# iwbn/flow-supervisor

Hardware: AMD Instinct MI355X
Metric: image-pairs/s fwd+bwd, 12 GRU iters, 436x1024 (higher is better)
Workload: dtype f32 (bf16x3 products); 1 GPU; RAFT full, 440x1024 (Sintel 436x1024 padded), 12 GRU iters, 4 pairs/GPU, train step = fwd + sequence loss + bwd + RCCL all-reduce + clip + AdamW; global_batch=4, parallelism=dp1, launch=hipGraph replay of the whole step

## Files before the change

### flow_supervisor_amd/csrc/conv_small.hip

```cpp
#include "common.hpp"
#include <cstddef>

namespace {


constexpr int SMALL_RUN = 16;
constexpr int SMALL_RUN_FWD = 8;
constexpr int SMALL_CHUNK = 8;

constexpr unsigned SM_OOB = 0x80000000u;
__device__ __forceinline__ __amdgpu_buffer_rsrc_t sm_rsrc(const void* p) {
  const uint64_t u = reinterpret_cast<uint64_t>(p);
  const unsigned lo = __builtin_amdgcn_readfirstlane((unsigned)u), hi = __builtin_amdgcn_readfirstlane((unsigned)(u >> 32));
  return __builtin_amdgcn_make_buffer_rsrc(reinterpret_cast<void*>((uint64_t)hi << 32 | lo), 0, 0x7fffffff, 0x00020000);
}

template <int KC, int NOUT, int KH, int KW>
__global__ __launch_bounds__(256) void conv_small_fwd_kernel(const float* __restrict__ x, int ld, int C,
                                                             const float* __restrict__ w, const float* __restrict__ bias,
                                                             float* __restrict__ out, int64_t obs, int64_t ocs, int64_t ops,
                                                             int B, int H, int W) {
  static_assert(KH == 3 && KW == 3, "sliding window written for 3 x 3");
  const int lane = threadIdx.x & 63;
  constexpr int taps = 9;
  const int HW = H * W;
  f32x4 wr[NOUT][taps][KC];
#pragma unroll
  for (int o = 0; o < NOUT; ++o)
#pragma unroll
    for (int kc = 0; kc < KC; ++kc) {
      const int c = kc * 256 + lane * 4;
      float buf[36];
#pragma unroll
      for (int q = 0; q < 9; ++q) {
        const f32x4 v = c < C ? *reinterpret_cast<const f32x4*>(w + ((int64_t)o * C + c) * taps + 4 * q) : f32x4{0.f, 0.f, 0.f, 0.f};
        buf[4 * q] = v[0]; buf[4 * q + 1] = v[1]; buf[4 * q + 2] = v[2]; buf[4 * q + 3] = v[3];
      }
#pragma unroll
      for (int t = 0; t < taps; ++t) wr[o][t][kc] = f32x4{buf[t], buf[9 + t], buf[18 + t], buf[27 + t]};
    }
  const int rpr = (W + SMALL_RUN_FWD - 1) / SMALL_RUN_FWD;
  const int64_t nrun = (int64_t)B * H * rpr;
  const int64_t wave = (int64_t)blockIdx.x * 4 + (threadIdx.x >> 6), nwaves = (int64_t)gridDim.x * 4;
  const f32x4 zero = {0.f, 0.f, 0.f, 0.f};
  for (int64_t run = wave; run < nrun; run += nwaves) {
    const int x0 = (int)(run % rpr) * SMALL_RUN_FWD;
    const int64_t by = run / rpr;
    const int y = (int)(by % H), b = (int)(by / H);
    const int n = W - x0 < SMALL_RUN_FWD ? W - x0 : SMALL_RUN_FWD;
    const float* img = x + (int64_t)b * HW * ld;
    const __amdgpu_buffer_rsrc_t rs = sm_rsrc(img);
    auto load_col = [&](int xs, f32x4 (&col)[3][KC]) {
#pragma unroll
      for (int r = 0; r < 3; ++r) {
        const int yy = y + r - 1;
        const bool in = (unsigned)yy < (unsigned)H && (unsigned)xs < (unsigned)W;
#pragma unroll
        for (int kc = 0; kc < KC; ++kc) {
          const int c = kc * 256 + lane * 4;
          col[r][kc] = __builtin_bit_cast(f32x4, __builtin_amdgcn_raw_buffer_load_b128(rs, (in && c < C) ? (unsigned)((yy * W + xs) * ld + c) * 4u : SM_OOB, 0, 0));
        }
      }
    };
    f32x4 c0[3][KC], c1[3][KC], cn[SMALL_RUN_FWD][3][KC];
    load_col(x0 - 1, c0);
    load_col(x0, c1);
#pragma unroll
    for (int i = 0; i < SMALL_RUN_FWD; ++i) load_col(x0 + i + 1, cn[i]);
#pragma unroll
    for (int i = 0; i < SMALL_RUN_FWD; ++i) {
      if (i < n) {
        float acc[NOUT];
#pragma unroll
        for (int o = 0; o < NOUT; ++o) {
          f32x4 a4 = zero;
#pragma unroll
          for (int r = 0; r < 3; ++r)
#pragma unroll
            for (int kc = 0; kc < KC; ++kc) {
              a4 += c0[r][kc] * wr[o][3 * r + 0][kc];
              a4 += c1[r][kc] * wr[o][3 * r + 1][kc];
              a4 += cn[i][r][kc] * wr[o][3 * r + 2][kc];
            }
          acc[o] = (a4[0] + a4[1]) + (a4[2] + a4[3]);
        }
#pragma unroll
        for (int o = 0; o < NOUT; ++o) {
#pragma unroll
          for (int sft = 32; sft > 0; sft >>= 1) acc[o] += __shfl_xor(acc[o], sft, 64);
        }
        if (lane == 0) {
          const int pix = y * W + x0 + i;
#pragma unroll
          for (int o = 0; o < NOUT; ++o) out[b * obs + o * ocs + pix * ops] = acc[o] + (bias ? bias[o] : 0.f);
        }
      }
#pragma unroll
      for (int r = 0; r < 3; ++r)
#pragma unroll
        for (int kc = 0; kc < KC; ++kc) { c0[r][kc] = c1[r][kc]; c1[r][kc] = cn[i][r][kc]; }
    }
  }
}

constexpr int SMALL_MAX_SEG = 16;
struct SmallWgradArgs {
  const float* dy[SMALL_MAX_SEG]; const float* x[SMALL_MAX_SEG]; int nseg;
  int ldy, ldx, C, B, H, W, KH, KW, Ktot;
  float* dwpk; float* dbias;
};

template <int KC, int NOUT, int KH, int KW>
__global__ __launch_bounds__(256) void conv_small_wgrad_kernel(SmallWgradArgs a) {
  __shared__ float red[4][64 * 4];
  const int lane = threadIdx.x & 63, wv = threadIdx.x >> 6;
  constexpr int taps = KH * KW;
  const int HW = a.H * a.W;
  f32x4 acc[NOUT][taps][KC];
#pragma unroll
  for (int o = 0; o < NOUT; ++o)
#pragma unroll
    for (int t = 0; t < taps; ++t)
#pragma unroll
      for (int kc = 0; kc < KC; ++kc) acc[o][t][kc] = f32x4{0.f, 0.f, 0.f, 0.f};
  float bsum[NOUT];
#pragma unroll
  for (int o = 0; o < NOUT; ++o) bsum[o] = 0.f;
  static_assert(KH == 3 && KW == 3, "sliding window written for 3 x 3");
  const int64_t wave = (int64_t)blockIdx.x * 4 + wv, nwaves = (int64_t)gridDim.x * 4;
  const auto* karg = (const char __attribute__((address_space(4)))*)__builtin_amdgcn_kernarg_segment_ptr();
  typedef const float* fptr;
  const int rpr = (a.W + SMALL_RUN - 1) / SMALL_RUN;
  const int64_t nrun = (int64_t)a.B * a.H * rpr;
  for (int seg = 0; seg < a.nseg; ++seg) {
    const float* dy = ((const fptr __attribute__((address_space(4)))*)(karg + offsetof(SmallWgradArgs, dy)))[seg];
    const float* x = ((const fptr __attribute__((address_space(4)))*)(karg + offsetof(SmallWgradArgs, x)))[seg];
    for (int64_t run = wave; run < nrun; run += nwaves) {
      const int x0 = (int)(run % rpr) * SMALL_RUN;
      const int64_t by = run / rpr;
      const int y = (int)(by % a.H), b = (int)(by / a.H);
      const int n = a.W - x0 < SMALL_RUN ? a.W - x0 : SMALL_RUN;
      const float* img = x + (int64_t)b * HW * a.ldx;
      const __amdgpu_buffer_rsrc_t rs = sm_rsrc(img);
      auto load_col = [&](int xs, f32x4 (&col)[3][KC]) {
#pragma unroll
        for (int r = 0; r < 3; ++r) {
          const int yy = y + r - 1;
          const bool in = (unsigned)yy < (unsigned)a.H && (unsigned)xs < (unsigned)a.W;
#pragma unroll
          for (int kc = 0; kc < KC; ++kc) {
            const int c = kc * 256 + lane * 4;
            col[r][kc] = __builtin_bit_cast(f32x4, __builtin_amdgcn_raw_buffer_load_b128(rs, (in && c < a.C) ? (unsigned)((yy * a.W + xs) * a.ldx + c) * 4u : SM_OOB, 0, 0));
          }
        }
      };
      f32x4 c0[3][KC], c1[3][KC];
      load_col(x0 - 1, c0);
      load_col(x0, c1);
      for (int i0 = 0; i0 < n; i0 += SMALL_CHUNK) {
        f32x4 cn[SMALL_CHUNK][3][KC];
        float g[SMALL_CHUNK][NOUT];
#pragma unroll
        for (int i = 0; i < SMALL_CHUNK; ++i) {
          load_col(x0 + i0 + i + 1, cn[i]);
          const int64_t m = (int64_t)b * HW + (int64_t)y * a.W + x0 + i0 + (i0 + i < n ? i : 0);
#pragma unroll
          for (int o = 0; o < NOUT; ++o) g[i][o] = i0 + i < n ? dy[m * a.ldy + o] : 0.f;
        }
#pragma unroll
        for (int i = 0; i < SMALL_CHUNK; ++i) {
#pragma unroll
          for (int o = 0; o < NOUT; ++o) bsum[o] += g[i][o];
#pragma unroll
          for (int r = 0; r < 3; ++r)
#pragma unroll
            for (int kc = 0; kc < KC; ++kc)
#pragma unroll
              for (int o = 0; o < NOUT; ++o) {
                acc[o][3 * r + 0][kc] += g[i][o] * c0[r][kc];
                acc[o][3 * r + 1][kc] += g[i][o] * c1[r][kc];
                acc[o][3 * r + 2][kc] += g[i][o] * cn[i][r][kc];
              }
#pragma unroll
          for (int r = 0; r < 3; ++r)
#pragma unroll
            for (int kc = 0; kc < KC; ++kc) { c0[r][kc] = c1[r][kc]; c1[r][kc] = cn[i][r][kc]; }
        }
      }
    }
  }
  const int cpad = ((a.C + 31) / 32) * 32;
#pragma unroll
  for (int o = 0; o < NOUT; ++o)
#pragma unroll
    for (int t = 0; t < taps; ++t) {
#pragma unroll
      for (int kc = 0; kc < KC; ++kc) {
        __syncthreads();
#pragma unroll
        for (int i = 0; i < 4; ++i) red[wv][lane * 4 + i] = acc[o][t][kc][i];
        __syncthreads();
        const int c = kc * 256 + threadIdx.x;
        if (c < a.C && threadIdx.x < 256) {
          const float s = (red[0][threadIdx.x] + red[1][threadIdx.x]) + (red[2][threadIdx.x] + red[3][threadIdx.x]);
          atomicAdd(a.dwpk + (int64_t)o * a.Ktot + t * cpad + c, s);
        }
      }
    }
  if (a.dbias && lane == 0) {
#pragma unroll
    for (int o = 0; o < NOUT; ++o) atomicAdd(a.dbias + o, bsum[o]);
  }
}

constexpr int SMALL_RUN_DG = 16;
template <int N>
__global__ __launch_bounds__(256) void conv_small_dgrad_kernel(const float* __restrict__ dy, int ldy, const float* __restrict__ w_oihw,
                                                               float* __restrict__ dx, int lddx, const float* __restrict__ relu_src,
                                                               int ldm, int C, int B, int H, int W) {
  static_assert(N == 2, "two output channels");
  const int lane = threadIdx.x & 63;
  const int c0 = lane * 4;
  const bool on = c0 < C;
  float wr[N][4][9];
#pragma unroll
  for (int o = 0; o < N; ++o)
#pragma unroll
    for (int k = 0; k < 4; ++k)
#pragma unroll
      for (int t = 0; t < 9; ++t) wr[o][k][t] = (on && c0 + k < C) ? w_oihw[((int64_t)o * C + c0 + k) * 9 + t] : 0.f;
  const int runs_per_row = (W + SMALL_RUN_DG - 1) / SMALL_RUN_DG;
  const int64_t nrun = (int64_t)B * H * runs_per_row;
  const int nwave = gridDim.x * 4;
  for (int64_t run = blockIdx.x * 4 + (threadIdx.x >> 6); run < nrun; run += nwave) {
    const int64_t ru = __builtin_amdgcn_readfirstlane((int)run);
    const int xr = (int)(ru % runs_per_row), row = (int)(ru / runs_per_row), y = row % H, b = row / H;
    const int x0 = xr * SMALL_RUN_DG, x1 = min(W, x0 + SMALL_RUN_DG);
    const float* dyb = dy + (int64_t)b * H * W * ldy;
    float g[3][3][N];
    auto col = [&](int x, float (&gc)[3][N]) {
#pragma unroll
      for (int j = 0; j < 3; ++j) {
        const int yy = y + j - 1;
        const bool ok = (unsigned)yy < (unsigned)H && (unsigned)x < (unsigned)W;
        const float* p = dyb + (int64_t)((ok ? yy : y) * W + (ok ? x : x0)) * ldy;
#pragma unroll
        for (int o = 0; o < N; ++o) gc[j][o] = ok ? p[o] : 0.f;
      }
    };
    col(x0 - 1, g[0]);
    col(x0, g[1]);
    for (int x = x0; x < x1; ++x) {
      col(x + 1, g[2]);
      if (on) {
        const int64_t pix = ((int64_t)b * H + y) * W + x;
        f32x4 acc = {0.f, 0.f, 0.f, 0.f};
#pragma unroll
        for (int ky = 0; ky < 3; ++ky)
#pragma unroll
          for (int kx = 0; kx < 3; ++kx)
#pragma unroll
            for (int o = 0; o < N; ++o) {
              const float gv = g[2 - kx][2 - ky][o];
#pragma unroll
              for (int k = 0; k < 4; ++k) acc[k] += wr[o][k][ky * 3 + kx] * gv;
            }
        if (relu_src) {
          const f32x4 m = gload4(relu_src + pix * ldm + c0);
#pragma unroll
          for (int k = 0; k < 4; ++k) acc[k] = m[k] > 0.f ? acc[k] : 0.f;
        }
        gstore4(dx + pix * lddx + c0, acc);
      }
#pragma unroll
      for (int j = 0; j < 3; ++j)
#pragma unroll
        for (int o = 0; o < N; ++o) { g[0][j][o] = g[1][j][o]; g[1][j][o] = g[2][j][o]; }
    }
  }
}

}

extern "C" int fsraft_conv_small_fwd(const float* x, int ld, int C, const float* w_oihw, const float* bias, float* out,
                                     int64_t obs, int64_t ocs, int64_t ops, int N, int B, int H, int W, int KH, int KW,
                                     hipStream_t s) {
  if (!x || !w_oihw || !out || N != 2 || C < 4 || C > 512 || C % 4 || ld % 4 || KH != 3 || KW != 3 || B < 1 || ((uintptr_t)w_oihw % 16)) return FS_ERR_ARG;
  const int64_t M = (int64_t)B * H * W;
  const int64_t nrun = (int64_t)B * H * ((W + SMALL_RUN_FWD - 1) / SMALL_RUN_FWD);
  int blocks = (int)((nrun + 3) / 4);
  if (blocks > 2048) blocks = 2048;
  (void)M;
  if (C <= 256) hipLaunchKernelGGL((conv_small_fwd_kernel<1, 2, 3, 3>), dim3(blocks), dim3(256), 0, s, x, ld, C, w_oihw, bias, out, obs, ocs, ops, B, H, W);
  else hipLaunchKernelGGL((conv_small_fwd_kernel<2, 2, 3, 3>), dim3(blocks), dim3(256), 0, s, x, ld, C, w_oihw, bias, out, obs, ocs, ops, B, H, W);
  return fs_launch_status();
}

extern "C" int fsraft_conv_small_wgrad(const float* const* dy, const float* const* x, int nseg, int ldy, int ldx, int C,
                                       float* dwpk, float* dbias, int N, int B, int H, int W, int KH, int KW, hipStream_t s) {
  if (!dy || !x || !dwpk || nseg < 1 || N != 2 || C < 4 || C > 512 || C % 4 || ldx % 4 || KH != 3 || KW != 3) return FS_ERR_ARG;
  for (int base = 0; base < nseg; base += SMALL_MAX_SEG) {
    SmallWgradArgs a{};
    a.nseg = nseg - base < SMALL_MAX_SEG ? nseg - base : SMALL_MAX_SEG;
    for (int i = 0; i < a.nseg; ++i) { a.dy[i] = dy[base + i]; a.x[i] = x[base + i]; if (!a.dy[i] || !a.x[i]) return FS_ERR_ARG; }
    a.ldy = ldy; a.ldx = ldx; a.C = C; a.B = B; a.H = H; a.W = W; a.KH = KH; a.KW = KW;
    a.Ktot = KH * KW * (((C + 31) / 32) * 32); a.dwpk = dwpk; a.dbias = dbias;
    if (C <= 256) hipLaunchKernelGGL((conv_small_wgrad_kernel<1, 2, 3, 3>), dim3(512), dim3(256), 0, s, a);
    else hipLaunchKernelGGL((conv_small_wgrad_kernel<2, 2, 3, 3>), dim3(512), dim3(256), 0, s, a);
    const int rc = fs_launch_status();
    if (rc) return rc;
  }
  return FS_OK;
}

extern "C" int fsraft_conv_small_dgrad(const float* dy, int ldy, const float* w_oihw, float* dx, int lddx, const float* relu_src, int ldm,
                                       int C, int N, int B, int H, int W, int KH, int KW, hipStream_t s) {
  if (!dy || !w_oihw || !dx || N != 2 || C < 4 || C > 256 || C % 4 || lddx % 4 || ldy < 2 || KH != 3 || KW != 3 || B < 1 ||
      ((uintptr_t)dx % 16) || (relu_src && (ldm % 4 || ((uintptr_t)relu_src % 16))))
    return FS_ERR_ARG;
  const int64_t nrun = (int64_t)B * H * ((W + SMALL_RUN_DG - 1) / SMALL_RUN_DG);
  if (nrun >= ((int64_t)1 << 31)) return FS_ERR_ARG;
  int blocks = (int)((nrun + 3) / 4);
  if (blocks > 4096) blocks = 4096;
  hipLaunchKernelGGL((conv_small_dgrad_kernel<2>), dim3(blocks), dim3(256), 0, s, dy, ldy, w_oihw, dx, lddx, relu_src, ldm, C, B, H, W);
  return fs_launch_status();
}
```

### flow_supervisor_amd/csrc/stem.hip

```cpp
#include "common.hpp"
#include "gemm_core_split.hpp"

namespace {

typedef unsigned u32x4 __attribute__((ext_vector_type(4)));

constexpr unsigned ST_OOB = 0x80000000u;
__device__ __forceinline__ __amdgpu_buffer_rsrc_t st_rsrc(const void* p) {
  const uint64_t u = reinterpret_cast<uint64_t>(p);
  const unsigned lo = __builtin_amdgcn_readfirstlane((unsigned)u), hi = __builtin_amdgcn_readfirstlane((unsigned)(u >> 32));
  return __builtin_amdgcn_make_buffer_rsrc(reinterpret_cast<void*>((uint64_t)hi << 32 | lo), 0, 0x7fffffff, 0x00020000);
}

constexpr int ST_TW = 32;
constexpr int ST_K = 192;
constexpr int ST_PC = 72;

struct StemArgs {
  const float* x;
  const float* w;
  const float* bias;
  float* out;
  const float* dy;
  float* scratch;
  int B, H, W, Ho, Wo, N, tx, ty, ntiles;
};

__device__ __forceinline__ void split1(float v, unsigned short& hi, unsigned short& lo) {
  const __bf16 h = (__bf16)v;
  hi = __builtin_bit_cast(unsigned short, h);
  lo = __builtin_bit_cast(unsigned short, (__bf16)(v - (float)h));
}

constexpr int SF_TH = 8, SF_PR = 2 * SF_TH + 6, SF_WPITCH = 400;
constexpr int SF_WBYTES = 64 * SF_WPITCH, SF_PBYTES = 3 * SF_PR * ST_PC * 2, SF_NCH = (3 * SF_PR * ST_PC + 511) / 512;

__global__ __launch_bounds__(512) void stem_fwd_kernel(const StemArgs a) {
  __shared__ __attribute__((aligned(16))) char lds[2 * SF_WBYTES + 4 * SF_PBYTES];
  char* wh = lds;
  char* wl = lds + SF_WBYTES;
  char* pbuf = lds + 2 * SF_WBYTES;
  const int lane = threadIdx.x & 63, wave = threadIdx.x >> 6, l31 = lane & 31, lh = lane >> 5;
  for (int e = threadIdx.x; e < 64 * ST_K; e += 512) {
    const int n = e / ST_K, k = e - n * ST_K, c = k >> 6, ky = (k >> 3) & 7, kx = k & 7;
    const float v = (n < a.N && ky < 7 && kx < 7) ? a.w[((n * 3 + c) * 7 + ky) * 7 + kx] : 0.f;
    unsigned short h, l;
    split1(v, h, l);
    *reinterpret_cast<unsigned short*>(wh + n * SF_WPITCH + k * 2) = h;
    *reinterpret_cast<unsigned short*>(wl + n * SF_WPITCH + k * 2) = l;
  }
  const int nb = (a.N + 31) >> 5;
  const int tpi = a.tx * a.ty;
  float rp[SF_NCH];
  int pos[SF_NCH];
#pragma unroll
  for (int j = 0; j < SF_NCH; ++j) {
    const int e = threadIdx.x + 512 * j;
    const int c = e / (SF_PR * ST_PC), r = e - c * (SF_PR * ST_PC), py = r / ST_PC, px = r - py * ST_PC;
    pos[j] = e < 3 * SF_PR * ST_PC ? c << 16 | py << 8 | px : -1;
  }
  auto fetch = [&](int tile) {
    const int b = tile / tpi, tr = tile - b * tpi, oy0 = (tr / a.tx) * SF_TH, ox0 = (tr % a.tx) * ST_TW;
    const int iy0 = 2 * oy0 - 3, ix0 = 2 * ox0 - 3;
    const __amdgpu_buffer_rsrc_t rs = st_rsrc(a.x + (int64_t)b * 3 * a.H * a.W);
#pragma unroll
    for (int j = 0; j < SF_NCH; ++j) {
      const int c = pos[j] >> 16, iy = iy0 + ((pos[j] >> 8) & 255), ix = ix0 + (pos[j] & 255);
      const bool ok = pos[j] >= 0 && (unsigned)iy < (unsigned)a.H && (unsigned)ix < (unsigned)a.W;
      rp[j] = __builtin_bit_cast(float, __builtin_amdgcn_raw_buffer_load_b32(rs, ok ? (unsigned)((c * a.H + iy) * a.W + ix) * 4u : ST_OOB, 0, 0));
    }
  };
  auto stage = [&](char* ph) {
#pragma unroll
    for (int j = 0; j < SF_NCH; ++j) {
      const int e = threadIdx.x + 512 * j;
      if (e < 3 * SF_PR * ST_PC) {
        unsigned short h, l;
        split1(rp[j], h, l);
        *reinterpret_cast<unsigned short*>(ph + e * 2) = h;
        *reinterpret_cast<unsigned short*>(ph + SF_PBYTES + e * 2) = l;
      }
    }
  };
  const float bv0 = (a.bias && l31 < a.N) ? a.bias[l31] : 0.f, bv1 = (a.bias && 32 + l31 < a.N) ? a.bias[32 + l31] : 0.f;
  if ((int)blockIdx.x < a.ntiles) {
    fetch(blockIdx.x);
    stage(pbuf);
  }
  __syncthreads();
  int it = 0;
  for (int tile = blockIdx.x; tile < a.ntiles; tile += gridDim.x, ++it) {
    const int b = tile / tpi, tr = tile - b * tpi, oy0 = (tr / a.tx) * SF_TH, ox0 = (tr % a.tx) * ST_TW;
    const char* ph = pbuf + (it & 1) * 2 * SF_PBYTES;
    const char* pl = ph + SF_PBYTES;
    const bool more = tile + (int)gridDim.x < a.ntiles;
    if (more) fetch(tile + gridDim.x);
    f32x16 acc[2];
#pragma unroll
    for (int j = 0; j < 2; ++j)
#pragma unroll
      for (int r = 0; r < 16; ++r) acc[j][r] = 0.f;
#pragma unroll
    for (int s = 0; s < ST_K / 16; ++s) {
      const int g = 2 * s + lh, c = g >> 3, ky = g & 7;
      const int ao = ((c * SF_PR + 2 * wave + ky) * ST_PC + 2 * l31) * 2;
      u32x4 ahv, alv;
#pragma unroll
      for (int i = 0; i < 4; ++i) {
        ahv[i] = *reinterpret_cast<const unsigned*>(ph + ao + 4 * i);
        alv[i] = *reinterpret_cast<const unsigned*>(pl + ao + 4 * i);
      }
      const bf16x8 ah = __builtin_bit_cast(bf16x8, ahv), al = __builtin_bit_cast(bf16x8, alv);
#pragma unroll
      for (int j = 0; j < 2; ++j) {
        if (j < nb) {
          const int bo = (j * 32 + l31) * SF_WPITCH + (s * 16 + lh * 8) * 2;
          const bf16x8 bh = *reinterpret_cast<const bf16x8*>(wh + bo), bl = *reinterpret_cast<const bf16x8*>(wl + bo);
          acc[j] = __builtin_amdgcn_mfma_f32_32x32x16_bf16(al, bh, acc[j], 0, 0, 0);
          acc[j] = __builtin_amdgcn_mfma_f32_32x32x16_bf16(ah, bl, acc[j], 0, 0, 0);
          acc[j] = __builtin_amdgcn_mfma_f32_32x32x16_bf16(ah, bh, acc[j], 0, 0, 0);
        }
      }
      if (s & 1) __builtin_amdgcn_sched_barrier(0);
    }
    if (more) stage(pbuf + ((it + 1) & 1) * 2 * SF_PBYTES);
    const int oy = oy0 + wave;
    if (oy < a.Ho) {
      const __amdgpu_buffer_rsrc_t ro = st_rsrc(a.out + (int64_t)b * a.Ho * a.Wo * a.N);
      const int oxl = ox0 + 4 * lh;
#pragma unroll
      for (int j = 0; j < 2; ++j) {
        const int n = j * 32 + l31;
        if (j < nb) {
          const float bv = j ? bv1 : bv0;
          const unsigned vo = n < a.N ? (unsigned)((oy * a.Wo + oxl) * a.N + n) * 4u : ST_OOB;
#pragma unroll
          for (int r = 0; r < 16; ++r) {
            const int dx = (r & 3) + 8 * (r >> 2);
            __builtin_amdgcn_raw_buffer_store_b32(__builtin_bit_cast(unsigned, acc[j][r] + bv), ro, oxl + dx < a.Wo ? vo : ST_OOB,
                                                  (unsigned)(dx * a.N) * 4u, 0);
          }
        }
      }
    }
    __syncthreads();
  }
}

constexpr int SW_TH = 1, SW_PX = SW_TH * ST_TW, SW_PR = 2 * SW_TH + 6, SW_NDY = SW_PX * 16 / 512;
constexpr int SW_DYPITCH = 64 * 2 + 64, SW_IMPITCH = ST_K * 2 + 64;
constexpr int SW_DYPLANE = SW_PX * SW_DYPITCH, SW_IMPLANE = SW_PX * SW_IMPITCH, SW_PATCH = 3 * SW_PR * ST_PC * 4;
constexpr int SW_NCHP = (3 * SW_PR * ST_PC + 511) / 512;

__global__ __launch_bounds__(512, 2) void stem_wgrad_kernel(const StemArgs a) {
  constexpr int SW_LDS = 2 * SW_DYPLANE + 2 * SW_IMPLANE + SW_PATCH > 64 * ST_K * 4 ? 2 * SW_DYPLANE + 2 * SW_IMPLANE + SW_PATCH : 64 * ST_K * 4;
  __shared__ __attribute__((aligned(16))) char lds[SW_LDS];
  char* dyh = lds;
  char* imh = lds + 2 * SW_DYPLANE;
  float* patch = reinterpret_cast<float*>(lds + 2 * SW_DYPLANE + 2 * SW_IMPLANE);
  const int lane = threadIdx.x & 63, wave = threadIdx.x >> 6;
  const int kg = wave >> 2, mi = wave & 1, ns = (wave >> 1) & 1;
  const int lh = lane >> 5, gb = (lane >> 4) & 1, q = (lane & 15) >> 2, p4 = lane & 3, l31 = lane & 31;
  const int tpi = a.tx * a.ty;
  f32x16 acc[3];
#pragma unroll
  for (int j = 0; j < 3; ++j)
#pragma unroll
    for (int r = 0; r < 16; ++r) acc[j][r] = 0.f;

  float rdy[4 * SW_NDY], rp[SW_NCHP];
  int pos[SW_NCHP];
#pragma unroll
  for (int j = 0; j < SW_NCHP; ++j) {
    const int e = threadIdx.x + 512 * j;
    const int c = e / (SW_PR * ST_PC), r = e - c * (SW_PR * ST_PC), py = r / ST_PC, pxx = r - py * ST_PC;
    pos[j] = e < 3 * SW_PR * ST_PC ? c << 16 | py << 8 | pxx : -1;
  }
  auto fetch = [&](int tile) {
    const int b = tile / tpi, tr = tile - b * tpi, oy0 = (tr / a.tx) * SW_TH, ox0 = (tr % a.tx) * ST_TW;
    const __amdgpu_buffer_rsrc_t rd = st_rsrc(a.dy + (int64_t)b * a.Ho * a.Wo * a.N);
#pragma unroll
    for (int c = 0; c < SW_NDY; ++c) {
      const int e = threadIdx.x + 512 * c, px = e >> 4, ch = (e & 15) * 4;
      const int oy = oy0 + (px >> 5), ox = ox0 + (px & 31);
      const bool ok = oy < a.Ho && ox < a.Wo && ch < a.N;
      const f32x4 v = __builtin_bit_cast(f32x4, __builtin_amdgcn_raw_buffer_load_b128(rd, ok ? (unsigned)((oy * a.Wo + ox) * a.N + ch) * 4u : ST_OOB, 0, 0));
      rdy[4 * c] = v[0]; rdy[4 * c + 1] = v[1]; rdy[4 * c + 2] = v[2]; rdy[4 * c + 3] = v[3];
    }
    const int iy0 = 2 * oy0 - 3, ix0 = 2 * ox0 - 3;
    const __amdgpu_buffer_rsrc_t rs = st_rsrc(a.x + (int64_t)b * 3 * a.H * a.W);
#pragma unroll
    for (int j = 0; j < SW_NCHP; ++j) {
      const int c = pos[j] >> 16, iy = iy0 + ((pos[j] >> 8) & 255), ix = ix0 + (pos[j] & 255);
      const bool ok = pos[j] >= 0 && (unsigned)iy < (unsigned)a.H && (unsigned)ix < (unsigned)a.W;
      rp[j] = __builtin_bit_cast(float, __builtin_amdgcn_raw_buffer_load_b32(rs, ok ? (unsigned)((c * a.H + iy) * a.W + ix) * 4u : ST_OOB, 0, 0));
    }
  };

  int tile = blockIdx.x;
  if (tile < a.ntiles) fetch(tile);
  for (; tile < a.ntiles; tile += gridDim.x) {
#pragma unroll
    for (int c = 0; c < SW_NDY; ++c) stage_convert_kmajor<64, SW_DYPITCH, SW_DYPLANE>(dyh, threadIdx.x + 512 * c, rdy + 4 * c);
#pragma unroll
    for (int j = 0; j < SW_NCHP; ++j)
      if (threadIdx.x + 512 * j < 3 * SW_PR * ST_PC) patch[threadIdx.x + 512 * j] = rp[j];
    __syncthreads();
    if (tile + (int)gridDim.x < a.ntiles) fetch(tile + gridDim.x);
    for (int it = threadIdx.x; it < SW_PX * 24; it += 512) {
      const int px = it / 24, g = it - px * 24, c = g >> 3, ky = g & 7;
      const float* src = patch + (c * SW_PR + 2 * (px >> 5) + ky) * ST_PC + 2 * (px & 31);
      float v[8];
#pragma unroll
      for (int i = 0; i < 8; ++i) v[i] = (ky < 7 && i < 7) ? src[i] : 0.f;
      uint2 h0, l0, h1, l1;
      split4(v, h0, l0);
      split4(v + 4, h1, l1);
      char* dst = imh + px * SW_IMPITCH + g * 16;
      *reinterpret_cast<uint4*>(dst) = make_uint4(h0.x, h0.y, h1.x, h1.y);
      *reinterpret_cast<uint4*>(dst + SW_IMPLANE) = make_uint4(l0.x, l0.y, l1.x, l1.y);
    }
    __syncthreads();
#pragma unroll
    for (int s = 0; s < SW_TH; ++s) {
      const int k0 = (kg * SW_TH + s) * 16;
      const char* Ap = dyh + (k0 + 8 * lh + q) * SW_DYPITCH + (mi * 32 + 16 * gb + 4 * p4) * 2;
      const bf16x8 ah = tr_frag(Ap, SW_DYPITCH), al = tr_frag(Ap + SW_DYPLANE, SW_DYPITCH);
#pragma unroll
      for (int j = 0; j < 3; ++j) {
        const char* Bp = imh + (k0 + 8 * lh + q) * SW_IMPITCH + ((3 * ns + j) * 32 + 16 * gb + 4 * p4) * 2;
        const bf16x8 bh = tr_frag(Bp, SW_IMPITCH), bl = tr_frag(Bp + SW_IMPLANE, SW_IMPITCH);
        acc[j] = __builtin_amdgcn_mfma_f32_32x32x16_bf16(al, bh, acc[j], 0, 0, 0);
        acc[j] = __builtin_amdgcn_mfma_f32_32x32x16_bf16(ah, bl, acc[j], 0, 0, 0);
        acc[j] = __builtin_amdgcn_mfma_f32_32x32x16_bf16(ah, bh, acc[j], 0, 0, 0);
      }
    }
    __syncthreads();
  }
  float* sum = reinterpret_cast<float*>(lds);
  __syncthreads();
  if (kg == 1) {
#pragma unroll
    for (int j = 0; j < 3; ++j)
#pragma unroll
      for (int r = 0; r < 16; ++r) sum[(mi * 32 + (r & 3) + 8 * (r >> 2) + 4 * lh) * ST_K + (3 * ns + j) * 32 + l31] = acc[j][r];
  }
  __syncthreads();
  if (kg == 0) {
    float* part = a.scratch + (int64_t)blockIdx.x * 64 * ST_K;
#pragma unroll
    for (int j = 0; j < 3; ++j)
#pragma unroll
      for (int r = 0; r < 16; ++r) {
        const int o = (mi * 32 + (r & 3) + 8 * (r >> 2) + 4 * lh) * ST_K + (3 * ns + j) * 32 + l31;
        part[o] = acc[j][r] + sum[o];
      }
  }
}

__global__ __launch_bounds__(256) void stem_wgrad_reduce_kernel(const float* __restrict__ scratch, int slots, float* __restrict__ dw, int N) {
  __shared__ float part[4][64];
  const int el = threadIdx.x & 63, pr = threadIdx.x >> 6;
  const int e = blockIdx.x * 64 + el;
  float s0 = 0.f, s1 = 0.f, s2 = 0.f, s3 = 0.f;
  if (e < N * 147) {
    const int n = e / 147, r = e - n * 147, c = r / 49, ky = (r % 49) / 7, kx = r % 7;
    const float* p = scratch + n * ST_K + (c * 8 + ky) * 8 + kx;
    int i = pr;
    for (; i + 60 < slots; i += 64) {
      float v[16];
#pragma unroll
      for (int j = 0; j < 16; ++j) v[j] = p[(int64_t)(i + 4 * j) * 64 * ST_K];
#pragma unroll
      for (int j = 0; j < 16; j += 4) { s0 += v[j]; s1 += v[j + 1]; s2 += v[j + 2]; s3 += v[j + 3]; }
    }
    for (; i + 12 < slots; i += 16) {
      s0 += p[(int64_t)i * 64 * ST_K];
      s1 += p[(int64_t)(i + 4) * 64 * ST_K];
      s2 += p[(int64_t)(i + 8) * 64 * ST_K];
      s3 += p[(int64_t)(i + 12) * 64 * ST_K];
    }
    for (; i < slots; i += 4) s0 += p[(int64_t)i * 64 * ST_K];
  }
  part[pr][el] = (s0 + s1) + (s2 + s3);
  __syncthreads();
  if (pr == 0 && e < N * 147) dw[e] = (part[0][el] + part[1][el]) + (part[2][el] + part[3][el]);
}

int stem_check(const void* x, const void* w, int B, int H, int W, int N) {
  if (!x || !w || B < 1 || H < 7 || W < 7 || (N != 32 && N != 64)) return FS_ERR_ARG;
  if ((int64_t)3 * H * W * 4 >= (int64_t)0x7fffffff || (int64_t)((H - 1) / 2 + 1) * ((W - 1) / 2 + 1) * N * 4 >= (int64_t)0x7fffffff) return FS_ERR_ARG;
  return FS_OK;
}

}

extern "C" int fsraft_stem_slots(void) { return 512; }

extern "C" int fsraft_stem7x7s2_fwd(const float* x, const float* w, const float* bias, float* out, int B, int H, int W, int N,
                                    hipStream_t stream) {
  const int rc = stem_check(x, w, B, H, W, N);
  if (rc || !out) return rc ? rc : FS_ERR_ARG;
  StemArgs a{};
  a.x = x; a.w = w; a.bias = bias; a.out = out;
  a.B = B; a.H = H; a.W = W; a.N = N;
  a.Ho = (H - 1) / 2 + 1; a.Wo = (W - 1) / 2 + 1;
  a.tx = ceil_div(a.Wo, ST_TW); a.ty = ceil_div(a.Ho, SF_TH);
  a.ntiles = B * a.tx * a.ty;
  const int grid = a.ntiles < 512 ? a.ntiles : 512;
  hipLaunchKernelGGL(stem_fwd_kernel, dim3(grid), dim3(512), 0, stream, a);
  return fs_launch_status();
}

extern "C" int fsraft_stem7x7s2_wgrad(const float* x, const float* dy, float* dw, float* scratch, int B, int H, int W, int N,
                                      hipStream_t stream) {
  const int rc = stem_check(x, dy, B, H, W, N);
  if (rc || !dw || !scratch || ((uintptr_t)dy & 15)) return rc ? rc : FS_ERR_ARG;
  StemArgs a{};
  a.x = x; a.dy = dy; a.scratch = scratch;
  a.B = B; a.H = H; a.W = W; a.N = N;
  a.Ho = (H - 1) / 2 + 1; a.Wo = (W - 1) / 2 + 1;
  a.tx = ceil_div(a.Wo, ST_TW); a.ty = ceil_div(a.Ho, SW_TH);
  a.ntiles = B * a.tx * a.ty;
  const int grid = a.ntiles < 512 ? a.ntiles : 512;
  hipLaunchKernelGGL(stem_wgrad_kernel, dim3(grid), dim3(512), 0, stream, a);
  int rc2 = fs_launch_status();
  if (rc2) return rc2;
  hipLaunchKernelGGL(stem_wgrad_reduce_kernel, dim3(ceil_div(N * 147, 64)), dim3(256), 0, stream, scratch, grid, dw, N);
  return fs_launch_status();
}
```

Measured before the change: 108.4 image-pairs/s.

## Remap blocks across XCDs, store conv outputs lane-parallel, template stem on N-blocks

```diff
diff --git a/flow_supervisor_amd/csrc/conv_small.hip b/flow_supervisor_amd/csrc/conv_small.hip
--- a/flow_supervisor_amd/csrc/conv_small.hip
+++ b/flow_supervisor_amd/csrc/conv_small.hip
@@ -9,6 +9,11 @@
 constexpr int SMALL_CHUNK = 8;
 
 constexpr unsigned SM_OOB = 0x80000000u;
+
+__device__ __forceinline__ unsigned sm_block() {
+  const unsigned g = gridDim.x, b = blockIdx.x;
+  return (g & 7u) ? b : (b & 7u) * (g >> 3) + (b >> 3);
+}
 __device__ __forceinline__ __amdgpu_buffer_rsrc_t sm_rsrc(const void* p) {
   const uint64_t u = reinterpret_cast<uint64_t>(p);
   const unsigned lo = __builtin_amdgcn_readfirstlane((unsigned)u), hi = __builtin_amdgcn_readfirstlane((unsigned)(u >> 32));
@@ -21,7 +26,10 @@
                                                              float* __restrict__ out, int64_t obs, int64_t ocs, int64_t ops,
                                                              int B, int H, int W) {
   static_assert(KH == 3 && KW == 3, "sliding window written for 3 x 3");
+  static_assert(NOUT * SMALL_RUN_FWD <= 64, "one lane per result of a run");
   const int lane = threadIdx.x & 63;
+  const int so = lane / SMALL_RUN_FWD, si = lane % SMALL_RUN_FWD;
+  const float sbias = (bias && so < NOUT) ? bias[so] : 0.f;
   constexpr int taps = 9;
   const int HW = H * W;
   f32x4 wr[NOUT][taps][KC];
@@ -41,7 +49,7 @@
     }
   const int rpr = (W + SMALL_RUN_FWD - 1) / SMALL_RUN_FWD;
   const int64_t nrun = (int64_t)B * H * rpr;
-  const int64_t wave = (int64_t)blockIdx.x * 4 + (threadIdx.x >> 6), nwaves = (int64_t)gridDim.x * 4;
+  const int64_t wave = (int64_t)sm_block() * 4 + (threadIdx.x >> 6), nwaves = (int64_t)gridDim.x * 4;
   const f32x4 zero = {0.f, 0.f, 0.f, 0.f};
   for (int64_t run = wave; run < nrun; run += nwaves) {
     const int x0 = (int)(run % rpr) * SMALL_RUN_FWD;
@@ -62,6 +70,7 @@
         }
       }
     };
+    float res = 0.f;
     f32x4 c0[3][KC], c1[3][KC], cn[SMALL_RUN_FWD][3][KC];
     load_col(x0 - 1, c0);
     load_col(x0, c1);
@@ -89,17 +98,15 @@
 #pragma unroll
           for (int sft = 32; sft > 0; sft >>= 1) acc[o] += __shfl_xor(acc[o], sft, 64);
         }
-        if (lane == 0) {
-          const int pix = y * W + x0 + i;
-#pragma unroll
-          for (int o = 0; o < NOUT; ++o) out[b * obs + o * ocs + pix * ops] = acc[o] + (bias ? bias[o] : 0.f);
-        }
+#pragma unroll
+        for (int o = 0; o < NOUT; ++o) res = lane == o * SMALL_RUN_FWD + i ? acc[o] : res;
       }
 #pragma unroll
       for (int r = 0; r < 3; ++r)
 #pragma unroll
         for (int kc = 0; kc < KC; ++kc) { c0[r][kc] = c1[r][kc]; c1[r][kc] = cn[i][r][kc]; }
     }
+    if (so < NOUT && si < n) out[b * obs + so * ocs + (int64_t)(y * W + x0 + si) * ops] = res + sbias;
   }
 }
 
@@ -127,7 +134,7 @@
 #pragma unroll
   for (int o = 0; o < NOUT; ++o) bsum[o] = 0.f;
   static_assert(KH == 3 && KW == 3, "sliding window written for 3 x 3");
-  const int64_t wave = (int64_t)blockIdx.x * 4 + wv, nwaves = (int64_t)gridDim.x * 4;
+  const int64_t wave = (int64_t)sm_block() * 4 + wv, nwaves = (int64_t)gridDim.x * 4;
   const auto* karg = (const char __attribute__((address_space(4)))*)__builtin_amdgcn_kernarg_segment_ptr();
   typedef const float* fptr;
   const int rpr = (a.W + SMALL_RUN - 1) / SMALL_RUN;
diff --git a/flow_supervisor_amd/csrc/stem.hip b/flow_supervisor_amd/csrc/stem.hip
--- a/flow_supervisor_amd/csrc/stem.hip
+++ b/flow_supervisor_amd/csrc/stem.hip
@@ -35,6 +35,7 @@
 constexpr int SF_TH = 8, SF_PR = 2 * SF_TH + 6, SF_WPITCH = 400;
 constexpr int SF_WBYTES = 64 * SF_WPITCH, SF_PBYTES = 3 * SF_PR * ST_PC * 2, SF_NCH = (3 * SF_PR * ST_PC + 511) / 512;
 
+template <int NB>
 __global__ __launch_bounds__(512) void stem_fwd_kernel(const StemArgs a) {
   __shared__ __attribute__((aligned(16))) char lds[2 * SF_WBYTES + 4 * SF_PBYTES];
   char* wh = lds;
@@ -49,7 +50,6 @@
     *reinterpret_cast<unsigned short*>(wh + n * SF_WPITCH + k * 2) = h;
     *reinterpret_cast<unsigned short*>(wl + n * SF_WPITCH + k * 2) = l;
   }
-  const int nb = (a.N + 31) >> 5;
   const int tpi = a.tx * a.ty;
   float rp[SF_NCH];
   int pos[SF_NCH];
@@ -95,9 +95,9 @@
     const char* pl = ph + SF_PBYTES;
     const bool more = tile + (int)gridDim.x < a.ntiles;
     if (more) fetch(tile + gridDim.x);
-    f32x16 acc[2];
-#pragma unroll
-    for (int j = 0; j < 2; ++j)
+    f32x16 acc[NB];
+#pragma unroll
+    for (int j = 0; j < NB; ++j)
 #pragma unroll
       for (int r = 0; r < 16; ++r) acc[j][r] = 0.f;
 #pragma unroll
@@ -112,14 +112,12 @@
       }
       const bf16x8 ah = __builtin_bit_cast(bf16x8, ahv), al = __builtin_bit_cast(bf16x8, alv);
 #pragma unroll
-      for (int j = 0; j < 2; ++j) {
-        if (j < nb) {
-          const int bo = (j * 32 + l31) * SF_WPITCH + (s * 16 + lh * 8) * 2;
-          const bf16x8 bh = *reinterpret_cast<const bf16x8*>(wh + bo), bl = *reinterpret_cast<const bf16x8*>(wl + bo);
-          acc[j] = __builtin_amdgcn_mfma_f32_32x32x16_bf16(al, bh, acc[j], 0, 0, 0);
-          acc[j] = __builtin_amdgcn_mfma_f32_32x32x16_bf16(ah, bl, acc[j], 0, 0, 0);
-          acc[j] = __builtin_amdgcn_mfma_f32_32x32x16_bf16(ah, bh, acc[j], 0, 0, 0);
-        }
+      for (int j = 0; j < NB; ++j) {
+        const int bo = (j * 32 + l31) * SF_WPITCH + (s * 16 + lh * 8) * 2;
+        const bf16x8 bh = *reinterpret_cast<const bf16x8*>(wh + bo), bl = *reinterpret_cast<const bf16x8*>(wl + bo);
+        acc[j] = __builtin_amdgcn_mfma_f32_32x32x16_bf16(al, bh, acc[j], 0, 0, 0);
+        acc[j] = __builtin_amdgcn_mfma_f32_32x32x16_bf16(ah, bl, acc[j], 0, 0, 0);
+        acc[j] = __builtin_amdgcn_mfma_f32_32x32x16_bf16(ah, bh, acc[j], 0, 0, 0);
       }
       if (s & 1) __builtin_amdgcn_sched_barrier(0);
     }
@@ -129,17 +127,15 @@
       const __amdgpu_buffer_rsrc_t ro = st_rsrc(a.out + (int64_t)b * a.Ho * a.Wo * a.N);
       const int oxl = ox0 + 4 * lh;
 #pragma unroll
-      for (int j = 0; j < 2; ++j) {
+      for (int j = 0; j < NB; ++j) {
         const int n = j * 32 + l31;
-        if (j < nb) {
-          const float bv = j ? bv1 : bv0;
-          const unsigned vo = n < a.N ? (unsigned)((oy * a.Wo + oxl) * a.N + n) * 4u : ST_OOB;
-#pragma unroll
-          for (int r = 0; r < 16; ++r) {
-            const int dx = (r & 3) + 8 * (r >> 2);
-            __builtin_amdgcn_raw_buffer_store_b32(__builtin_bit_cast(unsigned, acc[j][r] + bv), ro, oxl + dx < a.Wo ? vo : ST_OOB,
-                                                  (unsigned)(dx * a.N) * 4u, 0);
-          }
+        const float bv = j ? bv1 : bv0;
+        const unsigned vo = n < a.N ? (unsigned)((oy * a.Wo + oxl) * a.N + n) * 4u : ST_OOB;
+#pragma unroll
+        for (int r = 0; r < 16; ++r) {
+          const int dx = (r & 3) + 8 * (r >> 2);
+          __builtin_amdgcn_raw_buffer_store_b32(__builtin_bit_cast(unsigned, acc[j][r] + bv), ro, oxl + dx < a.Wo ? vo : ST_OOB,
+                                                (unsigned)(dx * a.N) * 4u, 0);
         }
       }
     }
@@ -308,7 +304,8 @@
   a.tx = ceil_div(a.Wo, ST_TW); a.ty = ceil_div(a.Ho, SF_TH);
   a.ntiles = B * a.tx * a.ty;
   const int grid = a.ntiles < 512 ? a.ntiles : 512;
-  hipLaunchKernelGGL(stem_fwd_kernel, dim3(grid), dim3(512), 0, stream, a);
+  if (N == 64) hipLaunchKernelGGL(stem_fwd_kernel<2>, dim3(grid), dim3(512), 0, stream, a);
+  else hipLaunchKernelGGL(stem_fwd_kernel<1>, dim3(grid), dim3(512), 0, stream, a);
   return fs_launch_status();
 }
 
```

New measurement: 109.0 image-pairs/s, median of 6. No clear change (+0.6%).
